# JuliaLinearAlgebra/IterativeSolvers.jl

Measured on AMD Instinct MI355X. Metric: cg_iters_per_sec, higher is better.
Workload: dtype f64; 1 GPU; cg! on 256^3 3D 7-point Laplacian (test/laplace_matrix.jl), fp64, hashed rhs, x0 = 0 (BASELINE.json configs[1]); n=16777216, nnz=117047296

## Files before the change

include/mik_dev.h:

```cpp
#include "mik.h"
#ifndef MIK_DEV_H
#define MIK_DEV_H
#ifdef __cplusplus
extern "C" {
#endif
enum {
    MIK_KNOB_LAYOUTS = 0,
    MIK_KNOB_CSR_KERNEL = 1,
    MIK_KNOB_SDIA_KERNEL = 2,
    MIK_KNOB_LONG_SEGMENT = 3,
    MIK_KNOB_UPLOAD = 4,
    MIK_KNOB_GS = 5,
    MIK_KNOB_TRANSPORT = 6,
    MIK_KNOB_NO_LOOKAHEAD = 7,
    MIK_KNOB_SOLVER_FORM = 8,
    MIK_KNOB_GS_TIMEOUT = 9,
    MIK_KNOB_CG_STEP = 10,
    MIK_KNOB_HOST_WAIT = 11,
    MIK_KNOB_MACHINE = 12,
    MIK_KNOB_COUNT = 13
};
int mik_set_tuning(int key, int value);
int mik_ctx_set_tuning(mik_ctx *ctx, int key, int value);
int mik_dev_gmres_form(const mik_gmres *it, int *single_launch, int *segments_per_workgroup, int *xcd_local_last, int *timeouts);
int mik_dev_dense_plan(const mik_dense *D, int adjoint, const void *x, const void *y, int *vec, int *streamed, int64_t *grid_x, int64_t *grid_y,
                       int64_t *chunks_or_batches, int64_t *segments);
int mik_dev_dense_block_plan(const mik_dense *D, int b, const void *X, int64_t ldx, const void *Y, int64_t ldy, int *vec, int *streamed,
                             int64_t *grid_x, int64_t *grid_y, int64_t *chunks, int *groups, int *last_width, int *vector_cols, int64_t *workspace_bytes);
int mik_dev_dense_block_min_width(mik_dense *D, int width);
int mik_dev_mgs_resident_shape(int *threads, int *register_rounds, int *lds_rounds);
int mik_dev_spmv_plan(const mik_csr *A, const void *x, int fuse_dot, int rb_begin, int rb_count, int skip_begin, int skip_end, char *kernel_name, int len,
                      int64_t *grid, int *launches, int *pre_longrows, int *post_rowdot);
int mik_dev_xwin_plan(int64_t n_blocks, const int *first_col, const int *last_col, const int *entries, int elem_size, int64_t n_cols,
                      int64_t total_entries, int *win_lo, int *span);
#ifdef __cplusplus
}
#endif
#endif
```

iterativesolvers.jl_amd/_lib.py:

```python
from __future__ import annotations

import ctypes as C
import os

import numpy as np

_HERE = os.path.dirname(os.path.abspath(__file__))
LIB_PATH = os.path.join(_HERE, "libmik.so")

MIK_OK = 0
MIK_F64, MIK_F32 = 0, 1
MIK_C64, MIK_C32 = 2, 3
MIK_SCALAR_REAL = 0x100
MIK_MGS, MIK_CGS, MIK_DGKS = 0, 1, 2
STATUS = {1: "invalid argument", 2: "HIP runtime error", 3: "dimension/dtype mismatch",
          4: "out of memory", 5: "not implemented", 6: "callback failed", 7: "norm outside the safely representable range",
          8: "singular"}


class MikError(RuntimeError):
    def __init__(self, code: int, where: str, detail: str = ""):
        self.code = code
        super().__init__(f"{where}: status {code} ({STATUS.get(code, '?')}) {detail}".rstrip())


_vp = C.c_void_p
_i64 = C.c_int64
_i64p = C.POINTER(C.c_int64)
_f64p = C.POINTER(C.c_double)
_ip = C.POINTER(C.c_int)

HALO_FN = C.CFUNCTYPE(C.c_int, C.c_void_p)
REDUCE_FN = C.CFUNCTYPE(C.c_int, C.c_void_p, C.c_int, C.c_int, C.c_void_p)


MUL_FN = C.CFUNCTYPE(C.c_int, C.c_void_p, C.c_void_p, C.c_void_p)
LDIV_FN = C.CFUNCTYPE(C.c_int, C.c_void_p, C.c_void_p, C.c_void_p)


class MikOperator(C.Structure):
    _fields_ = [("dtype", C.c_int), ("n", C.c_int64), ("csr", C.c_void_p), ("mul", MUL_FN), ("user", C.c_void_p)]


class MikPrecond(C.Structure):
    _fields_ = [("diag", C.c_void_p), ("ldiv", LDIV_FN), ("user", C.c_void_p)]


class MikDeviceInfo(C.Structure):
    _fields_ = [("device", C.c_int), ("compute_units", C.c_int), ("xcds", C.c_int), ("wavefront_size", C.c_int),
                ("lds_bytes_per_cu", C.c_int64), ("l2_bytes", C.c_int64), ("hbm_bytes", C.c_int64), ("arch", C.c_char * 64),
                ("planned_compute_units", C.c_int), ("planned_xcds", C.c_int), ("xcd_maps", C.c_int), ("resident_workgroup_cap", C.c_int),
                ("gs_single_launch_max_segments", C.c_int), ("gs_xcd_local_max_workgroups", C.c_int), ("sweep_grid_cap", C.c_int),
                ("mgs_resident_max_segments", C.c_int), ("reserved", C.c_int * 7)]


class MikPartition(C.Structure):
    _fields_ = [("rank", C.c_int), ("nranks", C.c_int), ("n_ext", C.c_int64), ("x_ext", C.c_void_p),
                ("send_idx", C.c_void_p), ("n_send", C.c_int64), ("send_buf", C.c_void_p),
                ("halo", HALO_FN), ("reduce", REDUCE_FN), ("user", C.c_void_p), ("link", C.c_void_p)]


class MikDensePlan(C.Structure):
    _fields_ = [("form", C.c_int), ("spin_limit", C.c_int)]


MIK_DENSE_AUTO, MIK_DENSE_PANEL, MIK_DENSE_CHAINED = 0, 1, 2


SIGNATURES = {
    "mik_abi_version": (C.c_int, []),
    "mik_device_count": (C.c_int, [_ip]),
    "mik_ctx_create": (C.c_int, [C.c_int, C.POINTER(_vp)]),
    "mik_ctx_destroy": (C.c_int, [_vp]),
    "mik_ctx_info": (C.c_int, [_vp, C.POINTER(MikDeviceInfo)]),
    "mik_dev_gmres_form": (C.c_int, [_vp, _ip, _ip, _ip, _ip]),
    "mik_dev_dense_plan": (C.c_int, [_vp, C.c_int, _vp, _vp, _ip, _ip, _i64p, _i64p, _i64p, _i64p]),
    "mik_dev_dense_block_plan": (C.c_int, [_vp, C.c_int, _vp, _i64, _vp, _i64, _ip, _ip, _i64p, _i64p, _i64p, _ip, _ip, _ip, _i64p]),
    "mik_dev_dense_block_min_width": (C.c_int, [_vp, C.c_int]),
    "mik_dev_mgs_resident_shape": (C.c_int, [_ip, _ip, _ip]),
    "mik_dev_spmv_plan": (C.c_int, [_vp, _vp, C.c_int, C.c_int, C.c_int, C.c_int, C.c_int, C.c_char_p, C.c_int, _i64p, _ip, _ip, _ip]),
    "mik_ctx_set_stream": (C.c_int, [_vp, _vp]),
    "mik_ctx_synchronize": (C.c_int, [_vp]),
    "mik_last_error": (C.c_char_p, [_vp]),
    "mik_reduce_shape": (C.c_int, [C.c_int, _ip, _ip]),
    "mik_spmv_dot_shape": (C.c_int, [_ip, _ip]),
    "mik_set_tuning": (C.c_int, [C.c_int, C.c_int]),
    "mik_ctx_set_tuning": (C.c_int, [_vp, C.c_int, C.c_int]),
    "mik_dev_xwin_plan": (C.c_int, [_i64, _ip, _ip, _ip, C.c_int, _i64, _i64, _ip, _ip]),
    "mik_spmv_long_row": (C.c_int, [_ip]),
    "mik_spmv_long_segment": (C.c_int, [_ip]),
    "mik_spmv_long_group": (C.c_int, [_ip]),
    "mik_malloc": (C.c_int, [_vp, C.c_size_t, C.POINTER(_vp)]),
    "mik_free": (C.c_int, [_vp, _vp]),
    "mik_memcpy_h2d": (C.c_int, [_vp, _vp, _vp, C.c_size_t]),
    "mik_memcpy_d2h": (C.c_int, [_vp, _vp, _vp, C.c_size_t]),
    "mik_copy": (C.c_int, [_vp, C.c_int, _i64, _vp, _vp]),
    "mik_fill": (C.c_int, [_vp, C.c_int, _i64, _vp, _vp]),
    "mik_csr_create": (C.c_int, [_vp, C.c_int, _i64, _i64, _i64, _i64p, _i64p, _vp, C.c_int, C.c_int,
                                 C.POINTER(_vp)]),
    "mik_csr_create_i32": (C.c_int, [_vp, C.c_int, _i64, _i64, _i64, C.POINTER(C.c_int32), C.POINTER(C.c_int32), _vp, C.c_int, C.c_int,
                                     C.POINTER(_vp)]),
    "mik_csr_destroy": (C.c_int, [_vp]),
    "mik_csr_layout": (C.c_int, [_vp, _ip]),
    "mik_csr_set_layout": (C.c_int, [_vp, C.c_int]),
    "mik_csr_stored_bytes": (C.c_int, [_vp, _i64p]),
    "mik_csr_compact": (C.c_int, [_vp]),
    "mik_spmv_kernel": (C.c_int, [_vp, C.c_char_p, C.c_int]),
    "mik_csr_info": (C.c_int, [_vp, _i64p, _i64p, _i64p, _ip]),
    "mik_spmv": (C.c_int, [_vp, _vp, _vp, _vp]),
    "mik_dot": (C.c_int, [_vp, C.c_int, _i64, _vp, _vp, _vp]),
    "mik_nrm2": (C.c_int, [_vp, C.c_int, _i64, _vp, _vp]),
    "mik_axpy": (C.c_int, [_vp, C.c_int, _i64, _vp, _vp, _vp]),
    "mik_xpby": (C.c_int, [_vp, C.c_int, _i64, _vp, _vp, _vp]),
    "mik_sub": (C.c_int, [_vp, C.c_int, _i64, _vp, _vp]),
    "mik_scal": (C.c_int, [_vp, C.c_int, _i64, _vp, _vp]),
    "mik_divide": (C.c_int, [_vp, C.c_int, _i64, _vp, _vp, _vp]),
    "mik_orthogonalize": (C.c_int, [_vp, C.c_int, _i64, C.c_int, _vp, _i64, _vp, _vp, _vp, C.c_int]),
    "mik_orthogonalize_vectors": (C.c_int, [_vp, C.c_int, _i64, C.c_int, C.POINTER(_vp), _vp, _vp, _vp]),
    "mik_gemv_n": (C.c_int, [_vp, C.c_int, _i64, C.c_int, _vp, _i64, _vp, _vp, _vp]),
    "mik_gemv_t": (C.c_int, [_vp, C.c_int, _i64, C.c_int, _vp, _i64, _vp, _vp]),
    "mik_lu_solve": (C.c_int, [C.c_int, _vp, _i64, C.c_int, _vp]),
    "mik_cg_create": (C.c_int, [_vp, _vp, _vp, _vp, _vp, _vp, _vp, _vp, C.c_double, C.c_double, _i64,
                                C.c_int, C.POINTER(_vp)]),
    "mik_cg_create_op": (C.c_int, [_vp, C.POINTER(MikOperator), C.POINTER(MikPrecond), _vp, _vp, _vp, _vp, _vp, C.c_double, C.c_double, _i64,
                                   C.c_int, C.POINTER(_vp)]),
    "mik_gmres_create_op": (C.c_int, [_vp, C.POINTER(MikOperator), C.POINTER(MikPrecond), C.POINTER(MikPrecond), _vp, _vp, C.c_double, C.c_double,
                                      C.c_int, _i64, C.c_int, C.c_int, C.POINTER(_vp)]),
    "mik_cg_destroy": (C.c_int, [_vp]),
    "mik_cg_fused_x": (C.c_int, [_vp, C.POINTER(C.c_int)]),
    "mik_cg_iterate": (C.c_int, [_vp, _i64, _f64p, _ip]),
    "mik_cg_iterate_many": (C.c_int, [_vp, _i64, _i64, _f64p, _i64p]),
    "mik_cg_state": (C.c_int, [_vp, _f64p, _f64p, _f64p, _i64p, _i64p, _ip]),
    "mik_gmres_create": (C.c_int, [_vp, _vp, _vp, _vp, _vp, _vp, C.c_double, C.c_double, C.c_int, _i64, C.c_int,
                                   C.c_int, C.POINTER(_vp)]),
    "mik_gmres_create_partitioned": (C.c_int, [_vp, _vp, _vp, _vp, _vp, _vp, C.c_double, C.c_double, C.c_int, _i64, C.c_int,
                                               C.c_int, C.POINTER(MikPartition), C.POINTER(_vp)]),
    "mik_gmres_destroy": (C.c_int, [_vp]),
    "mik_gmres_iterate": (C.c_int, [_vp, _i64, _f64p, _ip]),
    "mik_gmres_iterate_many": (C.c_int, [_vp, _i64, _i64, _f64p, _i64p]),
    "mik_gmres_state": (C.c_int, [_vp, _f64p, _f64p, _f64p, _ip, _i64p, _ip]),
    "mik_axpy_dot": (C.c_int, [_vp, C.c_int, _i64, _vp, _vp, _vp, _vp, _vp, C.c_int]),
    "mik_axpy2_nrm2": (C.c_int, [_vp, C.c_int, _i64, _vp, _vp, _vp, _vp, _vp, _vp, C.c_int]),
    "mik_cheb_direction": (C.c_int, [_vp, C.c_int, _i64, _vp, _vp, _vp, C.c_int, _vp]),
    "mik_minres_update": (C.c_int, [_vp, C.c_int, _i64, _vp, _vp, _vp, _vp, _vp, _vp, _vp, _vp, _vp, _vp, _vp, C.c_int]),
    "mik_gram": (C.c_int, [_vp, C.c_int, _i64, C.c_int, _vp, _i64, _vp]),
    "mik_bicgstab_mr_update": (C.c_int, [_vp, C.c_int, _i64, C.c_int, _vp, _i64, _vp, _i64, _vp, _vp, _vp]),
    "mik_bicgstab_create": (C.c_int, [_vp, _vp, C.c_int, _vp, _vp, _i64, _vp, _i64, _vp, _vp, C.POINTER(_vp)]),
    "mik_bicgstab_step": (C.c_int, [_vp, _vp]),
    "mik_bicgstab_destroy": (C.c_int, [_vp]),
    "mik_minres_create": (C.c_int, [_vp, _vp, _vp, _vp, _vp, _vp, _vp, _vp, _vp, C.c_double, C.c_int, C.POINTER(_vp)]),
    "mik_minres_step": (C.c_int, [_vp, _i64, _vp]),
    "mik_minres_proj_shape": (C.c_int, [_vp, _ip, _ip]),
    "mik_bicgstab_dot_shape": (C.c_int, [_vp, _ip, _ip]),
    "mik_minres_destroy": (C.c_int, [_vp]),
    "mik_xpby_nrm2": (C.c_int, [_vp, C.c_int, _i64, _vp, _vp, _vp, _vp]),
    "mik_lsqr_update": (C.c_int, [_vp, C.c_int, _i64, _vp, _vp, _vp, _vp, _vp, _vp, _vp]),
    "mik_lsmr_update": (C.c_int, [_vp, C.c_int, _i64, _vp, _vp, _vp, _vp, _vp, _vp, _vp, _vp]),
    "mik_axpy2_dot": (C.c_int, [_vp, C.c_int, _i64, _vp, _vp, _vp, _vp, _vp, _vp, _vp]),
    "mik_scal2": (C.c_int, [_vp, C.c_int, _i64, _vp, _vp, _vp, _vp]),
    "mik_qmr_update": (C.c_int, [_vp, C.c_int, _i64, _vp, _vp, _vp, _vp, _vp, _vp, _vp, _vp, _vp]),
    "mik_idrs_create": (C.c_int, [_vp, _vp, C.c_int, _vp, _vp, _vp, _i64, _vp, _i64, _vp, _i64, _vp, _vp, _vp, C.c_double, C.POINTER(_vp)]),
    "mik_idrs_step": (C.c_int, [_vp, C.c_int, _vp]),
    "mik_idrs_state": (C.c_int, [_vp, _vp, _vp, _vp]),
    "mik_idrs_destroy": (C.c_int, [_vp]),
    "mik_gather": (C.c_int, [_vp, C.c_int, _i64, _vp, _vp, _vp]),
    "mik_cgd_create": (C.c_int, [_vp, _vp, _vp, _vp, _vp, _vp, _vp, _vp, _i64, _vp, _vp, _vp, C.c_int, C.c_int,
                                 C.c_double, C.c_double, _i64, C.c_int, C.POINTER(_vp)]),
    "mik_cgd_destroy": (C.c_int, [_vp]),
    "mik_cgd_phase": (C.c_int, [_vp, C.c_int, _i64]),
    "mik_cgd_set_interior": (C.c_int, [_vp, _i64, _i64]),
    "mik_cgd_wait": (C.c_int, [_vp, _f64p, _f64p, _ip, _f64p, _i64, _i64p]),
    "mik_cgd_set_halo_plan": (C.c_int, [_vp, C.c_int, _ip, _i64p, _i64p, C.c_int, _ip, _i64p, _i64p]),
    "mik_cgd_halo_early": (C.c_int, [_vp, _ip, _i64p, _ip]),
    "mik_comm_unique_id": (C.c_int, [_vp]),
    "mik_comm_create": (C.c_int, [_vp, _vp, C.c_int, C.c_int, C.POINTER(_vp)]),
    "mik_comm_destroy": (C.c_int, [_vp]),
    "mik_comm_info": (C.c_int, [_vp, _ip, _ip, _ip]),
    "mik_comm_allgather_sum": (C.c_int, [_vp, C.c_int, C.c_int, _vp]),
    "mik_comm_halo": (C.c_int, [_vp, C.c_int, _vp, _vp, C.c_int, _ip, _i64p, _i64p, C.c_int, _ip, _i64p, _i64p]),
    "mik_cgd_set_comm": (C.c_int, [_vp, _vp]),
    "mik_comm_mailbox_export": (C.c_int, [_vp, _vp]),
    "mik_comm_mailbox_connect": (C.c_int, [_vp, _vp]),
    "mik_comm_mailbox_info": (C.c_int, [_vp, _ip, _ip]),
    "mik_cgd_ghost_export": (C.c_int, [_vp, _vp]),
    "mik_cgd_connect_ghosts": (C.c_int, [_vp, _vp, _i64p, _i64p]),
    "mik_plink_create": (C.c_int, [_vp, C.c_int, _i64, C.c_int, _ip, _i64p, _i64p, C.c_int, _ip, _i64p, _i64p, C.POINTER(_vp)]),
    "mik_plink_export": (C.c_int, [_vp, _vp]),
    "mik_plink_connect": (C.c_int, [_vp, _vp, _i64p, _i64p]),
    "mik_plink_info": (C.c_int, [_vp, _ip, _ip, _i64p]),
    "mik_plink_exchange": (C.c_int, [_vp, _vp, _vp]),
    "mik_plink_destroy": (C.c_int, [_vp]),
    "mik_cgd_init": (C.c_int, [_vp, _f64p, _f64p]),
    "mik_cgd_iterate_many": (C.c_int, [_vp, _i64, _i64, _f64p, _i64p]),
    "mik_cgd_group_init": (C.c_int, [C.POINTER(_vp), C.c_int, _f64p, _f64p]),
    "mik_cgd_group_iterate_many": (C.c_int, [C.POINTER(_vp), C.c_int, _i64, _i64, _f64p, _i64p]),
    "mik_cgd_group_release": (C.c_int, [C.POINTER(_vp), C.c_int]),
    "mik_hessenberg_ldiv": (C.c_int, [C.c_int, _vp, _i64, C.c_int, _vp]),
    "mik_givens": (C.c_int, [C.c_int, _vp, _vp, _vp]),
    "mik_time_spmv": (C.c_int, [_vp, _vp, _vp, _vp, C.c_int, C.c_int, _f64p]),
    "mik_cg_profile": (C.c_int, [_vp, C.c_int, _f64p, _i64p]),
    "mik_cgd_profile": (C.c_int, [_vp, C.c_int, _f64p, _i64p]),
    "mik_cg_profile_kernels": (C.c_int, [_vp, _f64p, _i64p]),
    "mik_stationary_create": (C.c_int, [_vp, _vp, _i64p, C.POINTER(_vp)]),
    "mik_stationary_destroy": (C.c_int, [_vp]),
    "mik_stationary_info": (C.c_int, [_vp, _i64p, _i64p, _i64p, _f64p]),
    "mik_diag_ldiv": (C.c_int, [_vp, _vp, _vp]),
    "mik_offdiag_mul": (C.c_int, [_vp, _vp, _vp, _vp, _vp]),
    "mik_gs_multiply": (C.c_int, [_vp, C.c_int, _vp, _vp, _vp, _vp, _vp]),
    "mik_forward_sub": (C.c_int, [_vp, _vp, _vp, _vp, _vp, C.c_int]),
    "mik_backward_sub": (C.c_int, [_vp, _vp, _vp, _vp, _vp, C.c_int]),
    "mik_dense_stationary_create": (C.c_int, [_vp, _vp, _i64, _i64, C.c_int, C.POINTER(MikDensePlan), _i64p, C.POINTER(_vp)]),
    "mik_dense_stationary_destroy": (C.c_int, [_vp]),
    "mik_dense_stationary_info": (C.c_int, [_vp, _i64p, _i64p, _i64p, _ip, _ip, _i64p]),
    "mik_dense_jacobi_step": (C.c_int, [_vp, _vp, _vp, _vp]),
    "mik_dense_gs_step": (C.c_int, [_vp, _vp, _vp]),
    "mik_dense_sor_step": (C.c_int, [_vp, _vp, _vp, _vp, _vp, C.c_int]),
    "mik_dense_ssor_step": (C.c_int, [_vp, _vp, _vp, _vp, _vp, C.c_int]),
    "mik_dense_mul_shape": (C.c_int, [_ip, _ip]),
    "mik_dense_mul_shape_for": (C.c_int, [C.c_int, _ip, _ip]),
    "mik_dense_create": (C.c_int, [_vp, C.c_int, _i64, _i64, _vp, _i64, C.POINTER(_vp)]),
    "mik_dense_destroy": (C.c_int, [_vp]),
    "mik_dense_mul": (C.c_int, [_vp, C.c_int, _vp, _vp]),
    "mik_dense_mm": (C.c_int, [_vp, C.c_int, _vp, _i64, _vp, _i64]),
    "mik_dense_block_reserve": (C.c_int, [_vp]),
    "mik_dense_block_shape": (C.c_int, [_ip]),
    "mik_dense_mul_fn": (C.c_int, [_vp, _vp, _vp]),
    "mik_dense_mul_adj_fn": (C.c_int, [_vp, _vp, _vp]),
    "mik_basis_rotate": (C.c_int, [_vp, C.c_int, _i64, C.c_int, C.c_int, _vp, _i64, _vp, _i64, _vp, _i64]),
    "mik_svdl_reorth": (C.c_int, [_vp, C.c_int, _i64, C.c_int, _vp, _i64, _vp, _vp, _vp, C.POINTER(C.c_int)]),
    "mik_spmm": (C.c_int, [_vp, _vp, C.c_int, _vp, _i64, _vp, _i64]),
    "mik_block_gram": (C.c_int, [_vp, C.c_int, _i64, C.c_int, C.c_int, _vp, _i64, _vp, _i64, _vp, _i64]),
    "mik_block_rdiv": (C.c_int, [_vp, C.c_int, _i64, C.c_int, _vp, _i64, _vp, _i64]),
    "mik_block_update": (C.c_int, [_vp, C.c_int, _i64, C.c_int, C.c_int, C.c_int, _vp, _i64, _vp, _i64, _vp, _i64, _vp, _i64, _vp, _i64, _vp, _i64]),
# ... 65 lines not shown
```

iterativesolvers.jl_amd/csrc/mik_core.hip:

```cpp
#include <algorithm>
#include <cmath>
#include <cstdarg>
#include <limits>
#include <new>

#include "mik_kernels.h"
#include "mik_spmv.h"
#include "mik_complex.h"
#include <algorithm>
#include <mutex>

#include "mik_sell.h"
#include "mik_jds.h"
#include <map>
#include <string>
#include <unordered_map>

thread_local std::string g_mik_create_error;
int g_mik_tuning[MIK_KNOB_COUNT] = {0};
static std::vector<mik_ctx *> g_mik_contexts;
static std::mutex g_mik_contexts_mu;

int mik_fail(mik_ctx *ctx, int code, const char *fmt, ...)
{
// ... 1474 lines not shown
    return lt;
}

template <typename T> static void spmv_go_sdiab(const SpmvPlan &p, const SpmvIO<T> &io)
{
    const mik_csr *A = io.A;
    with_consts([&](auto fd, auto cls) {
        constexpr int C = decltype(cls)::value;
        hipLaunchKernelGGL((k_spmv_sdiab<T, decltype(fd)::value, true, MIK_SDIAC_G, mik_sdiab_cls_ns(C), mik_sdiab_cls_cq(C)>), dim3(p.grid), dim3(MIK_BLOCK), 0,
                           io.ctx->stream, (int)A->n_rows, (int)A->n_cols, A->sdia_koff, p.rb0, p.nb, p.nfull, p.sshift, p.skip_at, p.skip_len,
                           (const SdiaSliceRec *)A->sdia_recs, (const SdiaPattern<T> *)A->sdia_pats, A->sdia_mask, io.x, io.y, io.seg_out, io.done);
    }, p.fd, SdiaCls{p.cls});
}

template <typename T> static void spmv_go_sdiab2(const SpmvPlan &p, const SpmvIO<T> &io)
{
    const mik_csr *A = io.A;
    with_consts([&](auto fd, auto cls) {
        constexpr int C = decltype(cls)::value;
        if constexpr (C >= 1)
            hipLaunchKernelGGL((k_spmv_sdiab2<T, decltype(fd)::value, true, mik_sdiab_cls_ns(C), mik_sdiab_cls_cq(C)>), dim3(p.grid), dim3(MIK_BLOCK), 0,
                               io.ctx->stream, (int)A->n_rows, (int)A->n_cols, A->sdia_koff, p.pb0, p.np, p.pfull, p.ps, p.nb_all,
                               (const SdiaSliceRec *)A->sdia_recs, (const SdiaPattern<T> *)A->sdia_pats, A->sdia_mask, io.x, io.y, io.seg_out, io.done,
                               io.ep_w(), io.ep_c(), io.ep_z());
    }, p.fd, SdiaCls{p.cls});
}

template <typename T> static void spmv_go_sdiac(const SpmvPlan &p, const SpmvIO<T> &io)
{
    const mik_csr *A = io.A;
    with_consts([&](auto fd) {
        hipLaunchKernelGGL((k_spmv_sdiac<T, decltype(fd)::value, true, MIK_SDIAC_G>), dim3(p.grid), dim3(MIK_BLOCK), 0, io.ctx->stream, (int)A->n_rows,
                           (int)A->n_cols, p.rb0, p.nb, p.map_mode, A->sdia_pat_id, (const SdiaPattern<T> *)A->sdia_pats, A->sdia_mask, io.x, io.y,
                           io.seg_out, io.done);
    }, p.fd);
}

template <typename T> static void spmv_go_sdiaw(const SpmvPlan &p, const SpmvIO<T> &io)
{
    const mik_csr *A = io.A;
    with_consts([&](auto fd) {
        if (p.kernel == SPMV_SDIAW2)
            hipLaunchKernelGGL((k_spmv_sdiaw2<T, decltype(fd)::value, true>), dim3(p.grid), dim3(MIK_BLOCK), 0, io.ctx->stream, (int)A->n_rows, (int)A->n_cols,
                               A->sdiaw_koff, p.pb0, p.np, p.pmode, p.nb_all, A->sdiaw_pat_id, (const SdiawPattern<T> *)A->sdiaw_pats, A->sdiaw_mask,
                               (const uint4 *)A->sdiaw_uz, io.x, io.y, io.seg_out, io.done);
        else
            hipLaunchKernelGGL((k_spmv_sdiaw<T, decltype(fd)::value, true>), dim3(p.grid), dim3(MIK_BLOCK), 0, io.ctx->stream, (int)A->n_rows, A->sdiaw_koff,
                               p.rb0, p.nb, p.map_mode, A->sdiaw_pat_id, (const SdiawPattern<T> *)A->sdiaw_pats, A->sdiaw_mask, io.x, io.y, io.seg_out,
                               io.done);
    }, p.fd);
}

template <typename T> static void spmv_go_sdia(const SpmvPlan &p, const SpmvIO<T> &io)
{
    const mik_csr *A = io.A;
    with_consts([&](auto fd) {
        hipLaunchKernelGGL((k_spmv_sdia<T, decltype(fd)::value, true>), dim3(p.grid), dim3(MIK_BLOCK), 0, io.ctx->stream, (int)A->n_rows, (int)A->n_cols, p.rb0,
                           p.nb, p.map_mode, A->sdia_ptr, A->sdia_off, A->sdia_tri, A->sdia_mask, (const T *)A->sdia_val, io.x, io.y, io.seg_out, io.done);
    }, p.fd);
}

template <typename T> static void spmv_go_jds(const SpmvPlan &p, const SpmvIO<T> &io)
{
    const mik_csr *A = io.A;
    using IV = typename WideVec<T>::idx;
    using VV = typename WideVec<T>::val;
    with_consts([&](auto fd, auto mg) {
        if constexpr (!(decltype(fd)::value && decltype(mg)::value))
            hipLaunchKernelGGL((k_spmv_jds<T, decltype(fd)::value, true, decltype(mg)::value>), dim3(p.grid), dim3(MIK_BLOCK), 0, io.ctx->stream, (int)A->n_rows,
                               p.rb0, A->jds_ptr, A->jds_len, (const IV *)A->jds_col, (const VV *)A->jds_val, io.x, io.y, io.seg_out, io.done, p.nlb,
                               spmv_long_tab(A), A->col, (const T *)A->val, io.ep_w(), io.ep_c(), io.ep_z());
    }, p.fd, p.merge);
}

template <typename T> static void spmv_go_rowgather(const SpmvPlan &p, const SpmvIO<T> &io)
{
    const mik_csr *A = io.A;
    with_consts([&](auto fd) {
        hipLaunchKernelGGL((k_spmv_rowgather<T, decltype(fd)::value, true>), dim3(p.grid), dim3(MIK_BLOCK), 0, io.ctx->stream, (int)A->n_rows, p.rb0, p.nb,
                           p.map_mode, A->rowptr, A->col, (const T *)A->val, io.x, io.y, io.seg_out, io.done, A->is_long, io.ep_w(), io.ep_c(), io.ep_z());
    }, p.fd);
}

template <typename T> static void spmv_go_rowblock(const SpmvPlan &p, const SpmvIO<T> &io)
{
    const mik_csr *A = io.A;
    with_consts([&](auto fd, auto mg, auto nt, auto xw, auto rp) {
        if constexpr (!(decltype(fd)::value && decltype(mg)::value))
            hipLaunchKernelGGL((k_spmv_rowblock<T, decltype(fd)::value, decltype(nt)::value, true, decltype(mg)::value, decltype(xw)::value, decltype(rp)::value>),
                               dim3(p.grid), dim3(MIK_BLOCK), p.lds, io.ctx->stream, (int)A->n_rows, p.nb, p.map_mode, A->rowptr, A->col, (const T *)A->val,
                               io.x, io.y, io.seg_out, io.done, A->is_long, p.nlb, spmv_long_tab(A), (const int *)A->xwin_lo, A->xwin_span,
                               (const unsigned char *)A->rperm, (p.merge && p.long_win) ? (const int *)A->long_win : (const int *)nullptr, p.lw_launch,
                               io.ep_w(), io.ep_c(), io.ep_z());
    }, p.fd, p.merge, p.nt_rb, p.xwin, p.rp);
}

template <typename T> static int spmv_run(const SpmvPlan &p, const SpmvIO<T> &io)
{
    mik_ctx *ctx = io.ctx;
    const mik_csr *A = io.A;
    if (p.rc != MIK_OK) return mik_fail(ctx, p.rc, "%s", p.refusal);
    if (p.empty) return MIK_OK;
    if (p.pre_longrows) {
        hipLaunchKernelGGL((k_spmv_longrows<T>), dim3(p.nlb), dim3(MIK_BLOCK), p.pre_lds, ctx->stream, spmv_long_tab(A), A->col, (const T *)A->val, io.x, io.y,
                           io.done, p.long_win ? (const int *)A->long_win : (const int *)nullptr, A->long_lw);
        MIK_LAUNCH_CHECK(ctx);
    }
    switch (p.kernel) {
    case SPMV_ROWGATHER: spmv_go_rowgather<T>(p, io); break;
    case SPMV_ROWBLOCK: spmv_go_rowblock<T>(p, io); break;
    case SPMV_JDS: spmv_go_jds<T>(p, io); break;
    case SPMV_SDIA: spmv_go_sdia<T>(p, io); break;
    case SPMV_SDIAC: spmv_go_sdiac<T>(p, io); break;
    case SPMV_SDIAB: spmv_go_sdiab<T>(p, io); break;
    case SPMV_SDIAB2: spmv_go_sdiab2<T>(p, io); break;
    case SPMV_SDIAW: case SPMV_SDIAW2: spmv_go_sdiaw<T>(p, io); break;
    }
    MIK_LAUNCH_CHECK(ctx);
    if (p.post_rowdot) {
        hipLaunchKernelGGL((k_rowdot<T>), dim3(p.nb_all), dim3(MIK_BLOCK), 0, ctx->stream, (int)A->n_rows, io.x, (const T *)io.y, io.seg_out, io.done);
        MIK_LAUNCH_CHECK(ctx);
    }
    return MIK_OK;
}

template <typename T>
int mik_spmv_launch_range(mik_ctx *ctx, const mik_csr *A, const T *x, T *y, bool fuse_dot, T *seg_out, const int *done, int rb_begin,
                          int rb_count)
{
    return spmv_run<T>(spmv_plan(A, sizeof(T), mik_aligned16(x), fuse_dot, rb_begin, rb_count, SPMV_NO_SKIP, 0, spmv_ep_armed(ctx)), {ctx, A, x, y, seg_out, done});
}

template <typename T>
int mik_spmv_launch(mik_ctx *ctx, const mik_csr *A, const T *x, T *y, bool fuse_dot, T *seg_out, const int *done)
{
    return mik_spmv_launch_range<T>(ctx, A, x, y, fuse_dot, seg_out, done, 0, -1);
}

template <typename T>
int mik_spmv_launch_outside(mik_ctx *ctx, const mik_csr *A, const T *x, T *y, bool fuse_dot, T *seg_out, const int *done, int skip_begin, int skip_end)
{
    SpmvPlan p[2];
    const int np = spmv_plan_outside(A, sizeof(T), mik_aligned16(x), fuse_dot, skip_begin, skip_end, spmv_ep_armed(ctx), p);
    for (int i = 0; i < np; ++i) MIK_TRY(spmv_run<T>(p[i], {ctx, A, x, y, seg_out, done}));
    return MIK_OK;
}
template int mik_spmv_launch_outside<double>(mik_ctx *, const mik_csr *, const double *, double *, bool, double *, const int *, int, int);
template int mik_spmv_launch_outside<float>(mik_ctx *, const mik_csr *, const float *, float *, bool, float *, const int *, int, int);
template int mik_spmv_launch<double>(mik_ctx *, const mik_csr *, const double *, double *, bool, double *, const int *);
template int mik_spmv_launch<float>(mik_ctx *, const mik_csr *, const float *, float *, bool, float *, const int *);
template int mik_spmv_launch_range<double>(mik_ctx *, const mik_csr *, const double *, double *, bool, double *, const int *, int, int);
template int mik_spmv_launch_range<float>(mik_ctx *, const mik_csr *, const float *, float *, bool, float *, const int *, int, int);

extern "C" int mik_spmv(mik_ctx *ctx, const mik_csr *A, const void *x, void *y)
{
    if (!ctx || !A || !x || !y) return MIK_ERR_INVALID;
    if (x == y) return mik_fail(ctx, MIK_ERR_INVALID, "mik_spmv: x and y must not alias");
    if (mik_is_complex(A->dtype)) return mik_c_spmv(ctx, A, x, y);
    return A->dtype == MIK_F64 ? mik_spmv_launch<double>(ctx, A, (const double *)x, (double *)y, false, nullptr, nullptr)
                               : mik_spmv_launch<float>(ctx, A, (const float *)x, (float *)y, false, nullptr, nullptr);
}

template <typename T>
static int time_spmv_impl(mik_ctx *ctx, const mik_csr *A, const void *x, void *y, int fused, int reps, double *avg_ms)
{
    int rc = mik_ensure_partials(ctx, sizeof(T) * (size_t)std::max<int64_t>((A->n_rows + MIK_BLOCK - 1) / MIK_BLOCK, 1));
    if (rc) return rc;
    hipEvent_t e0, e1;
    MIK_HIP(ctx, hipEventCreate(&e0));
    MIK_HIP(ctx, hipEventCreate(&e1));
    MIK_HIP(ctx, hipEventRecord(e0, ctx->stream));
    for (int i = 0; i < reps; ++i) {
        rc = mik_spmv_launch<T>(ctx, A, (const T *)x, (T *)y, fused != 0, (T *)ctx->partials, nullptr);
        if (rc) return rc;
    }
    MIK_HIP(ctx, hipEventRecord(e1, ctx->stream));
    MIK_HIP(ctx, hipEventSynchronize(e1));
    float ms = 0.f;
    MIK_HIP(ctx, hipEventElapsedTime(&ms, e0, e1));
    (void)hipEventDestroy(e0);
    (void)hipEventDestroy(e1);
    *avg_ms = (double)ms / reps;
    return MIK_OK;
}

extern "C" int mik_time_spmv(mik_ctx *ctx, const mik_csr *A, const void *x, void *y, int fused_dot, int reps, double *avg_ms)
{
    if (!ctx || !A || !x || !y || reps <= 0 || !avg_ms) return MIK_ERR_INVALID;
    if (mik_is_complex(A->dtype)) return mik_c_time_spmv(ctx, A, x, y, reps, avg_ms);
    return A->dtype == MIK_F64 ? time_spmv_impl<double>(ctx, A, x, y, fused_dot, reps, avg_ms)
                               : time_spmv_impl<float>(ctx, A, x, y, fused_dot, reps, avg_ms);
}

template <typename T> static int reduce_to_host(mik_ctx *ctx, int64_t n, T *out)
{
    const int64_t nseg = mik_nseg<T>(n);
    hipLaunchKernelGGL((k_finalize_store<T>), dim3(1), dim3(MIK_FIN_THREADS), 0, ctx->stream, (const T *)ctx->partials, nseg,
                       (int64_t)0, (T *)ctx->coef, (const int *)nullptr);
    MIK_LAUNCH_CHECK(ctx);
    return mik_read_scalars<T>(ctx, (const T *)ctx->coef, 1, out);
}

template <typename T> static int norm_from_sumsq(mik_ctx *ctx, int64_t n, const T *x, T t, T *out)
{
    if (mik_nrm_in_range(t)) { *out = (T)std::sqrt(t); return MIK_OK; }
    return mik_safe_norm_slow<T>(ctx, n, x, out);
}

template <typename T> int mik_safe_norm_slow(mik_ctx *ctx, int64_t n, const T *x, T *out)
{
    if (n <= 0) { *out = T(0); return MIK_OK; }
    T *scr = (T *)((unsigned char *)ctx->coef + mik_ctx::COEF_SAFE_SLOT);
    const int grid = (int)std::min<int64_t>((n + MIK_BLOCK - 1) / MIK_BLOCK, 1024);
    MIK_TRY(mik_ensure_partials(ctx, sizeof(T) * (size_t)std::max<int64_t>(std::max<int64_t>(mik_nseg<T>(n), grid), 1)));
    hipLaunchKernelGGL((k_amax<T>), dim3(grid), dim3(MIK_BLOCK), 0, ctx->stream, n, x, (T *)ctx->partials);
    MIK_LAUNCH_CHECK(ctx);
    hipLaunchKernelGGL((k_amax<T>), dim3(1), dim3(MIK_BLOCK), 0, ctx->stream, (int64_t)grid, (const T *)ctx->partials, scr);
    MIK_LAUNCH_CHECK(ctx);
    T amax;
    MIK_TRY(mik_read_scalars<T>(ctx, scr, 1, &amax));
    T sc, sinv;
    if (!mik_nrm_scale(amax, sc, sinv)) { *out = amax; return MIK_OK; }
    OpScaledSq<T> op{x, sc};
    MIK_TRY((launch_map<T>(ctx, n, op, mik_aligned16(x), (T *)ctx->partials, nullptr)));
    hipLaunchKernelGGL((k_finalize_store<T>), dim3(1), dim3(MIK_FIN_THREADS), 0, ctx->stream, (const T *)ctx->partials, mik_nseg<T>(n),
                       (int64_t)0, scr, (const int *)nullptr);
    MIK_LAUNCH_CHECK(ctx);
    T t2;
    MIK_TRY(mik_read_scalars<T>(ctx, scr, 1, &t2));
    *out = (T)std::sqrt(t2) * sinv;
    return MIK_OK;
}
template int mik_safe_norm_slow<double>(mik_ctx *, int64_t, const double *, double *);
template int mik_safe_norm_slow<float>(mik_ctx *, int64_t, const float *, float *);

template <typename T> static int dot_impl(mik_ctx *ctx, int64_t n, const void *x, const void *y, void *out, bool nrm)
{
    int rc = mik_ensure_partials(ctx, sizeof(T) * (size_t)std::max<int64_t>(mik_nseg<T>(n), 1));
    if (rc) return rc;
    OpDot<T> op{(const T *)x, (const T *)y};
    rc = launch_map<T>(ctx, n, op, mik_aligned16(x) && mik_aligned16(y), (T *)ctx->partials, nullptr);
    if (rc) return rc;
    T v;
    MIK_TRY(reduce_to_host<T>(ctx, n, &v));
    if (!nrm) { *(T *)out = v; return MIK_OK; }
    return norm_from_sumsq<T>(ctx, n, (const T *)x, v, (T *)out);
}

extern "C" int mik_dot(mik_ctx *ctx, int dtype, int64_t n, const void *x, const void *y, void *out)
{
    if (!ctx || n < 0 || !out || (n && (!x || !y))) return MIK_ERR_INVALID;
    if (mik_is_complex(dtype)) return mik_c_dot(ctx, dtype, n, x, y, out);
    return dtype == MIK_F64 ? dot_impl<double>(ctx, n, x, y, out, false) : dot_impl<float>(ctx, n, x, y, out, false);
}

extern "C" int mik_nrm2(mik_ctx *ctx, int dtype, int64_t n, const void *x, void *out)
{
    if (!ctx || n < 0 || !out || (n && !x)) return MIK_ERR_INVALID;
    if (mik_is_complex(dtype)) return mik_nrm2(ctx, mik_real_dtype(dtype), 2 * n, x, out);
    return dtype == MIK_F64 ? dot_impl<double>(ctx, n, x, x, out, true) : dot_impl<float>(ctx, n, x, x, out, true);
}

extern "C" int mik_axpy(mik_ctx *ctx, int dtype, int64_t n, const void *alpha, const void *x, void *y)
{
    if (!ctx || n < 0 || !alpha || (n && (!x || !y))) return MIK_ERR_INVALID;
    if (mik_is_complex(dtype & ~MIK_SCALAR_REAL))
        return (dtype & MIK_SCALAR_REAL) ? mik_axpy(ctx, mik_real_dtype(dtype & ~MIK_SCALAR_REAL), 2 * n, alpha, x, y) : mik_c_axpy(ctx, dtype, n, alpha, x, y);
    const bool vec = mik_aligned16(x) && mik_aligned16(y);
    if (dtype == MIK_F64) { OpAxpy<double> op{(const double *)x, (double *)y, coef_val(*(const double *)alpha)}; return launch_map<double>(ctx, n, op, vec, (double *)nullptr, nullptr); }
    if (dtype == MIK_F32) { OpAxpy<float> op{(const float *)x, (float *)y, coef_val(*(const float *)alpha)}; return launch_map<float>(ctx, n, op, vec, (float *)nullptr, nullptr); }
    return MIK_ERR_INVALID;
}

extern "C" int mik_xpby(mik_ctx *ctx, int dtype, int64_t n, const void *x, const void *beta, void *y)
{
    if (!ctx || n < 0 || !beta || (n && (!x || !y))) return MIK_ERR_INVALID;
    if (mik_is_complex(dtype & ~MIK_SCALAR_REAL))
        return (dtype & MIK_SCALAR_REAL) ? mik_xpby(ctx, mik_real_dtype(dtype & ~MIK_SCALAR_REAL), 2 * n, x, beta, y) : mik_c_xpby(ctx, dtype, n, x, beta, y);
    const bool vec = mik_aligned16(x) && mik_aligned16(y);
    if (dtype == MIK_F64) { OpXpby<double> op{(const double *)x, (double *)y, coef_val(*(const double *)beta)}; return launch_map<double>(ctx, n, op, vec, (double *)nullptr, nullptr); }
    if (dtype == MIK_F32) { OpXpby<float> op{(const float *)x, (float *)y, coef_val(*(const float *)beta)}; return launch_map<float>(ctx, n, op, vec, (float *)nullptr, nullptr); }
    return MIK_ERR_INVALID;
}

extern "C" int mik_sub(mik_ctx *ctx, int dtype, int64_t n, const void *x, void *y)
{
    if (!ctx || n < 0 || (n && (!x || !y))) return MIK_ERR_INVALID;
    if (mik_is_complex(dtype)) return mik_sub(ctx, mik_real_dtype(dtype), 2 * n, x, y);
    const bool vec = mik_aligned16(x) && mik_aligned16(y);
    if (dtype == MIK_F64) { OpSub<double> op{(const double *)x, (double *)y}; return launch_map<double>(ctx, n, op, vec, (double *)nullptr, nullptr); }
    if (dtype == MIK_F32) { OpSub<float> op{(const float *)x, (float *)y}; return launch_map<float>(ctx, n, op, vec, (float *)nullptr, nullptr); }
    return MIK_ERR_INVALID;
}

extern "C" int mik_scal(mik_ctx *ctx, int dtype, int64_t n, const void *alpha, void *x)
{
    if (!ctx || n < 0 || !alpha || (n && !x)) return MIK_ERR_INVALID;
    if (mik_is_complex(dtype & ~MIK_SCALAR_REAL))
        return (dtype & MIK_SCALAR_REAL) ? mik_scal(ctx, mik_real_dtype(dtype & ~MIK_SCALAR_REAL), 2 * n, alpha, x) : mik_c_scal(ctx, dtype, n, alpha, x);
    const bool vec = mik_aligned16(x);
    if (dtype == MIK_F64) { OpScal<double> op{(double *)x, coef_val(*(const double *)alpha)}; return launch_map<double>(ctx, n, op, vec, (double *)nullptr, nullptr); }
    if (dtype == MIK_F32) { OpScal<float> op{(float *)x, coef_val(*(const float *)alpha)}; return launch_map<float>(ctx, n, op, vec, (float *)nullptr, nullptr); }
    return MIK_ERR_INVALID;
}

template <typename T>
// ... 221 lines not shown
```

iterativesolvers.jl_amd/csrc/mik_spmv.h:

```cpp
#pragma once
#include "mik_internal.h"

#ifdef __HIPCC__

template <bool NT, typename U> __device__ __forceinline__ U ld_stream(const U *p)
{
    return NT ? __builtin_nontemporal_load(p) : *p;
}
template <bool NT, typename U> __device__ __forceinline__ void st_stream(U *p, U v)
{
    if (NT) __builtin_nontemporal_store(v, p); else *p = v;
}

typedef double mik_f64x2 __attribute__((ext_vector_type(2)));
typedef float mik_f32x4 __attribute__((ext_vector_type(4)));
typedef int mik_i32x2 __attribute__((ext_vector_type(2)));
typedef int mik_i32x4 __attribute__((ext_vector_type(4)));
template <typename T> struct WideVec;
template <> struct WideVec<double> { using val = mik_f64x2; using idx = mik_i32x2; };
template <> struct WideVec<float>  { using val = mik_f32x4; using idx = mik_i32x4; };

__device__ __forceinline__ int spmv_block_map(int b, int nb, int mode)
{
    if (mode == 1) return xcd_remap(b, nb);
// ... 152 lines not shown
    constexpr int TILE = MIK_SPMV_TILE * (int)(8 / sizeof(T));
    constexpr int VW = WIDE ? VT<T>::W : 1;
    constexpr int PER = TILE / (MIK_BLOCK * VW);
    extern __shared__ __attribute__((aligned(16))) unsigned char mik_dyn_lds[];
    T *prod = reinterpret_cast<T *>(mik_dyn_lds);
    T *lds4 = prod + TILE + 8;

    const int t = threadIdx.x;
    int bid = blockIdx.x;
    if (MERGE_LONG) {
        const bool spread = lw < 0;
        if (spread) lw = -lw;
        unsigned which = (unsigned)bid;
        bool is_long = bid < nlb;
        if (spread) {
            const unsigned total = gridDim.x;
            const unsigned before = (unsigned)(((unsigned long long)bid * (unsigned)nlb + total - 1) / total);
            const unsigned upto = (unsigned)(((unsigned long long)(bid + 1) * (unsigned)nlb + total - 1) / total);
            is_long = upto > before;
            which = is_long ? before : (unsigned)bid - before;
        } else if (!is_long) which = (unsigned)(bid - nlb);
        if (is_long) {
            const int lwlo = long_win ? long_win[which] : -1;
            if (lwlo >= 0) spmv_long_window<T>(x, prod, lwlo, lw);
            spmv_longrow_wave<T>((int)which * (MIK_BLOCK / 64) + (t >> 6), lt, col, val, x, y, prod, lwlo >= 0 ? lwlo : 0, lwlo >= 0 ? lw : 0);
            return;
        }
        bid = (int)which;
    }
    const int rb = spmv_block_map(bid, nb, map_mode);
    const int r0 = rb * MIK_BLOCK;
    const int tr = RPERM ? (int)rperm[r0 + t] : t;
    const int r = r0 + tr;
    int ks = 0, ke = 0;
    if (r < n) { ks = rowptr[r]; ke = rowptr[r + 1]; }
    const int kb = rowptr[r0] & ~(VW - 1);
    const int kend = rowptr[min(r0 + MIK_BLOCK, n)];
    T *xw = lds4 + 16 / (int)sizeof(T) * ((4 * (int)sizeof(T) + 15) / 16);
    int wlo = 0;
    if (XWIN) {
        constexpr int XP = 1024 / (int)sizeof(T);
        wlo = win_lo[rb];
        if (kb < kend && wlo >= 0)
            for (int piece = t >> 6; piece * XP < win_span; piece += MIK_BLOCK / 64)
                __builtin_amdgcn_global_load_lds((const __attribute__((address_space(1))) void *)(x + wlo + piece * XP + (t & 63) * (16 / (int)sizeof(T))),
                                                 (__attribute__((address_space(3))) void *)(xw + piece * XP), 16, 0, 0);
    }

    T acc = T(0);
    for (int kc = kb; kc < kend; kc += TILE) {
        const int cnt = min(TILE, kend - kc);
        if (WIDE) {
            using VV = typename WideVec<T>::val;
            using IV = typename WideVec<T>::idx;
            VV v[PER];
            IV c[PER];
#pragma unroll
            for (int i = 0; i < PER; ++i) {
                const int j = VW * (t + MIK_BLOCK * i);
                if (j < cnt) {
                    v[i] = ld_stream<NT>(reinterpret_cast<const VV *>(val + kc + j));
                    c[i] = ld_stream<NT>(reinterpret_cast<const IV *>(col + kc + j));
                }
            }
            if (XWIN && wlo >= 0) {
                if (kc == kb) {
                    asm volatile("s_waitcnt vmcnt(0)" ::: "memory");
                    __syncthreads();
                }
#pragma unroll
                for (int i = 0; i < PER; ++i) {
                    const int j = VW * (t + MIK_BLOCK * i);
                    if (j < cnt) {
#pragma unroll
                        for (int e = 0; e < VW; ++e) {
                            const unsigned o = min((unsigned)(c[i][e] - wlo), (unsigned)(win_span - 1));
                            prod[j + e] = v[i][e] * xw[o];
                        }
                    }
                }
            } else {
#pragma unroll
                for (int i = 0; i < PER; ++i) {
                    const int j = VW * (t + MIK_BLOCK * i);
                    if (j < cnt) {
                        T xv[VW];
#pragma unroll
                        for (int e = 0; e < VW; ++e) xv[e] = x[c[i][e]];
#pragma unroll
                        for (int e = 0; e < VW; ++e) prod[j + e] = v[i][e] * xv[e];
                    }
                }
            }
        } else {
            T v[PER];
            int c[PER];
#pragma unroll
            for (int i = 0; i < PER; ++i) {
                const int j = t + MIK_BLOCK * i;
                if (j < cnt) { v[i] = ld_stream<NT>(val + kc + j); c[i] = ld_stream<NT>(col + kc + j); }
            }
#pragma unroll
            for (int i = 0; i < PER; ++i) {
                const int j = t + MIK_BLOCK * i;
                if (j < cnt) prod[j] = v[i] * x[c[i]];
            }
        }
        __syncthreads();
        int a = max(ks, kc) - kc;
        int len = min(ke, kc + cnt) - kc - a;
        for (; len >= 8; len -= 8, a += 8) {
            T q[8];
#pragma unroll
            for (int i = 0; i < 8; ++i) q[i] = prod[a + i];
#pragma unroll
            for (int i = 0; i < 8; ++i) acc = acc + q[i];
        }
        if (len > 0) {
            T q[8];
#pragma unroll
            for (int i = 0; i < 8; ++i) q[i] = prod[a + i];
#pragma unroll
            for (int i = 0; i < 8; ++i) {
                const T s2 = acc + q[i];
                acc = i < len ? s2 : acc;
            }
        }
        __syncthreads();
    }
    if (FUSE_DOT && ep_w && r < n) { const T te = *ep_c * ep_w[r]; acc = acc + te; }
    if (is_long && r < n && is_long[r]) acc = y[r];
    else if (r < n) st_stream<NT>(y + r, acc);
    if (FUSE_DOT) {
        T p = T(0);
        if (r < n) p = (ep_z ? ep_z[r] : x[r]) * acc;
        if (RPERM) {
            prod[tr] = p;
            __syncthreads();
            p = prod[t];
        }
        T tot = block_tree_256(p, lds4);
        if (t == 0) seg_out[rb] = tot;
    }
}

template <typename T, bool FUSE_DOT, bool NT>
__global__ __launch_bounds__(MIK_BLOCK, 6) void k_spmv_rowgather(int n, int rb0, int nb, int map_mode, const int *__restrict__ rowptr,
                                                              const int *__restrict__ col, const T *__restrict__ val,
                                                              const T *__restrict__ x, T *__restrict__ y, T *__restrict__ seg_out,
                                                              const int *__restrict__ done, const unsigned char *__restrict__ is_long,
                                                              const T *__restrict__ ep_w = nullptr, const T *__restrict__ ep_c = nullptr,
                                                             const T *__restrict__ ep_z = nullptr)
{
    if (done && *done) return;
    constexpr int TILE = MIK_SPMV_TILE;
    constexpr int VW = VT<T>::W;
    constexpr int VP = 1024 / (int)sizeof(T);
    constexpr int CP = 256;
    __shared__ __attribute__((aligned(16))) T sval[TILE];
    __shared__ __attribute__((aligned(16))) int scol[TILE];
    __shared__ T lds4[4];

    const int t = threadIdx.x, lane = t & 63, wv = t >> 6;
    const int rb = rb0 + spmv_block_map((int)blockIdx.x, nb, map_mode);
    const int r0 = rb * MIK_BLOCK;
    const int r = r0 + t;
    int ks = 0, ke = 0;
    if (r < n) { ks = rowptr[r]; ke = rowptr[r + 1]; }
    const int kb = rowptr[r0] & ~3;
    const int kend = rowptr[min(r0 + MIK_BLOCK, n)];

    T acc = T(0);
    for (int kc = kb; kc < kend; kc += TILE) {
        const int cnt = min(TILE, kend - kc);
#pragma unroll
        for (int p = 0; p < TILE / VP / 4; ++p) {
            const int piece = wv + 4 * p;
            if (piece * VP < cnt)
                __builtin_amdgcn_global_load_lds((const __attribute__((address_space(1))) void *)(val + kc + piece * VP + lane * VW),
                                                 (__attribute__((address_space(3))) void *)(sval + piece * VP), 16, 0, NT ? 2 : 0);
        }
#pragma unroll
        for (int p = 0; p < TILE / CP / 4; ++p) {
            const int piece = wv + 4 * p;
            if (piece * CP < cnt)
                __builtin_amdgcn_global_load_lds((const __attribute__((address_space(1))) void *)(col + kc + piece * CP + lane * 4),
                                                 (__attribute__((address_space(3))) void *)(scol + piece * CP), 16, 0, NT ? 2 : 0);
        }
        asm volatile("s_waitcnt vmcnt(0)" ::: "memory");
        __syncthreads();
        int a = max(ks, kc) - kc;
        int len = min(ke, kc + cnt) - kc - a;
        while (len > 0) {
            T q[8];
            int cc[8];
#pragma unroll
            for (int i = 0; i < 8; ++i) {
                const int s = min(a + i, TILE - 1);
                cc[i] = scol[s];
                q[i] = sval[s];
            }
#pragma unroll
            for (int i = 0; i < 8; ++i) {
                const T xv = x[i < len ? cc[i] : 0];
                q[i] = q[i] * xv;
            }
#pragma unroll
            for (int i = 0; i < 8; ++i)
                if (i < len) acc = acc + q[i];
            a += 8;
            len -= 8;
        }
        if (kc + TILE < kend) __syncthreads();
    }
    if (FUSE_DOT && ep_w && r < n) { const T te = *ep_c * ep_w[r]; acc = acc + te; }
    if (is_long && r < n && is_long[r]) acc = y[r];
    else if (r < n) st_stream<NT>(y + r, acc);
    if (FUSE_DOT) {
        T p = T(0);
        if (r < n) p = (ep_z ? ep_z[r] : x[r]) * acc;
        T tot = block_tree_256(p, lds4);
        if (t == 0) seg_out[rb] = tot;
    }
}

#endif
```

Baseline: 2166 iters/s.

## Pipeline rowgather SpMV tile loads: issue col before val, overlap x gather

The row-gather SpMV kernel now issues the column-index LDS loads before the value loads and waits only for the column loads. It then starts the first batch of x gathers before waiting for the value tile, so value loading overlaps with the dependent x reads. Row pointers, the done flag and the fused-dot operand are loaded up front, pinned in registers, and the dot reuses the prefetched x value. The change also adds a C/Python entry point, mik_dev_spmv_run, for launching SpMV ranges directly. In exchange it relies on hand-managed vmcnt/barrier sequencing and adds an extra barrier per tile, which raises the risk of correctness bugs.

```diff
diff --git a/include/mik_dev.h b/include/mik_dev.h
--- a/include/mik_dev.h
+++ b/include/mik_dev.h
@@ -31,6 +31,8 @@
 int mik_dev_mgs_resident_shape(int *threads, int *register_rounds, int *lds_rounds);
 int mik_dev_spmv_plan(const mik_csr *A, const void *x, int fuse_dot, int rb_begin, int rb_count, int skip_begin, int skip_end, char *kernel_name, int len,
                       int64_t *grid, int *launches, int *pre_longrows, int *post_rowdot);
+int mik_dev_spmv_run(mik_ctx *ctx, const mik_csr *A, const void *x, void *y, int fuse_dot, void *seg_out, int rb_begin, int rb_count, int skip_begin,
+                     int skip_end);
 int mik_dev_xwin_plan(int64_t n_blocks, const int *first_col, const int *last_col, const int *entries, int elem_size, int64_t n_cols,
                       int64_t total_entries, int *win_lo, int *span);
 #ifdef __cplusplus
diff --git a/iterativesolvers.jl_amd/_lib.py b/iterativesolvers.jl_amd/_lib.py
--- a/iterativesolvers.jl_amd/_lib.py
+++ b/iterativesolvers.jl_amd/_lib.py
@@ -79,6 +79,7 @@
     "mik_dev_dense_block_min_width": (C.c_int, [_vp, C.c_int]),
     "mik_dev_mgs_resident_shape": (C.c_int, [_ip, _ip, _ip]),
     "mik_dev_spmv_plan": (C.c_int, [_vp, _vp, C.c_int, C.c_int, C.c_int, C.c_int, C.c_int, C.c_char_p, C.c_int, _i64p, _ip, _ip, _ip]),
+    "mik_dev_spmv_run": (C.c_int, [_vp, _vp, _vp, _vp, C.c_int, _vp, C.c_int, C.c_int, C.c_int, C.c_int]),
     "mik_ctx_set_stream": (C.c_int, [_vp, _vp]),
     "mik_ctx_synchronize": (C.c_int, [_vp]),
     "mik_last_error": (C.c_char_p, [_vp]),
diff --git a/iterativesolvers.jl_amd/csrc/mik_core.hip b/iterativesolvers.jl_amd/csrc/mik_core.hip
--- a/iterativesolvers.jl_amd/csrc/mik_core.hip
+++ b/iterativesolvers.jl_amd/csrc/mik_core.hip
@@ -1650,6 +1650,24 @@
 template int mik_spmv_launch_range<double>(mik_ctx *, const mik_csr *, const double *, double *, bool, double *, const int *, int, int);
 template int mik_spmv_launch_range<float>(mik_ctx *, const mik_csr *, const float *, float *, bool, float *, const int *, int, int);
 
+template <typename T>
+static int dev_spmv_run(mik_ctx *ctx, const mik_csr *A, const void *x, void *y, bool fuse_dot, void *seg_out, int rb_begin, int rb_count, int skip_begin,
+                        int skip_end)
+{
+    if (skip_begin < 0) return mik_spmv_launch_range<T>(ctx, A, (const T *)x, (T *)y, fuse_dot, (T *)seg_out, nullptr, rb_begin, rb_count);
+    return mik_spmv_launch_outside<T>(ctx, A, (const T *)x, (T *)y, fuse_dot, (T *)seg_out, nullptr, skip_begin, skip_end);
+}
+
+extern "C" int mik_dev_spmv_run(mik_ctx *ctx, const mik_csr *A, const void *x, void *y, int fuse_dot, void *seg_out, int rb_begin, int rb_count,
+                                int skip_begin, int skip_end)
+{
+    if (!ctx || !A || !x || !y || (fuse_dot && !seg_out)) return MIK_ERR_INVALID;
+    if (x == y) return mik_fail(ctx, MIK_ERR_INVALID, "mik_dev_spmv_run: x and y must not alias");
+    MIK_REFUSE_COMPLEX(ctx, A, "mik_dev_spmv_run");
+    return A->dtype == MIK_F64 ? dev_spmv_run<double>(ctx, A, x, y, fuse_dot != 0, seg_out, rb_begin, rb_count, skip_begin, skip_end)
+                               : dev_spmv_run<float>(ctx, A, x, y, fuse_dot != 0, seg_out, rb_begin, rb_count, skip_begin, skip_end);
+}
+
 extern "C" int mik_spmv(mik_ctx *ctx, const mik_csr *A, const void *x, void *y)
 {
     if (!ctx || !A || !x || !y) return MIK_ERR_INVALID;
diff --git a/iterativesolvers.jl_amd/csrc/mik_spmv.h b/iterativesolvers.jl_amd/csrc/mik_spmv.h
--- a/iterativesolvers.jl_amd/csrc/mik_spmv.h
+++ b/iterativesolvers.jl_amd/csrc/mik_spmv.h
@@ -328,7 +328,6 @@
                                                               const T *__restrict__ ep_w = nullptr, const T *__restrict__ ep_c = nullptr,
                                                              const T *__restrict__ ep_z = nullptr)
 {
-    if (done && *done) return;
     constexpr int TILE = MIK_SPMV_TILE;
     constexpr int VW = VT<T>::W;
     constexpr int VP = 1024 / (int)sizeof(T);
@@ -337,25 +336,27 @@
     __shared__ __attribute__((aligned(16))) int scol[TILE];
     __shared__ T lds4[4];
 
-    const int t = threadIdx.x, lane = t & 63, wv = t >> 6;
+    const int t = threadIdx.x, lane = t & 63;
+    const int wv = __builtin_amdgcn_readfirstlane(t >> 6);
     const int rb = rb0 + spmv_block_map((int)blockIdx.x, nb, map_mode);
     const int r0 = rb * MIK_BLOCK;
     const int r = r0 + t;
-    int ks = 0, ke = 0;
-    if (r < n) { ks = rowptr[r]; ke = rowptr[r + 1]; }
-    const int kb = rowptr[r0] & ~3;
+    const int rl = min(r, n - 1);
+    int ks = rowptr[rl], ke = rowptr[rl + 1];
+    T xr = T(0);
+    if (FUSE_DOT) xr = (ep_z ? ep_z : x)[rl];
+    const int kfirst = rowptr[r0];
     const int kend = rowptr[min(r0 + MIK_BLOCK, n)];
+    const int stop = *(done ? done : rowptr);
+    if (FUSE_DOT) asm volatile("" :: "v"(ks), "v"(ke), "v"(xr), "s"(kfirst), "s"(kend), "s"(stop), "s"(col), "s"(val), "s"(x), "s"(y));
+    else asm volatile("" :: "v"(ks), "v"(ke), "s"(kfirst), "s"(kend), "s"(stop), "s"(col), "s"(val), "s"(x), "s"(y));
+    if (done && stop) return;
+    if (r >= n) ks = ke = 0;
+    const int kb = kfirst & ~3;
 
     T acc = T(0);
     for (int kc = kb; kc < kend; kc += TILE) {
         const int cnt = min(TILE, kend - kc);
-#pragma unroll
-        for (int p = 0; p < TILE / VP / 4; ++p) {
-            const int piece = wv + 4 * p;
-            if (piece * VP < cnt)
-                __builtin_amdgcn_global_load_lds((const __attribute__((address_space(1))) void *)(val + kc + piece * VP + lane * VW),
-                                                 (__attribute__((address_space(3))) void *)(sval + piece * VP), 16, 0, NT ? 2 : 0);
-        }
 #pragma unroll
         for (int p = 0; p < TILE / CP / 4; ++p) {
             const int piece = wv + 4 * p;
@@ -363,10 +364,50 @@
                 __builtin_amdgcn_global_load_lds((const __attribute__((address_space(1))) void *)(col + kc + piece * CP + lane * 4),
                                                  (__attribute__((address_space(3))) void *)(scol + piece * CP), 16, 0, NT ? 2 : 0);
         }
-        asm volatile("s_waitcnt vmcnt(0)" ::: "memory");
-        __syncthreads();
+        int nv = 0;
+#pragma unroll
+        for (int p = 0; p < TILE / VP / 4; ++p) {
+            const int piece = wv + 4 * p;
+            if (piece * VP < cnt) {
+                __builtin_amdgcn_global_load_lds((const __attribute__((address_space(1))) void *)(val + kc + piece * VP + lane * VW),
+                                                 (__attribute__((address_space(3))) void *)(sval + piece * VP), 16, 0, NT ? 2 : 0);
+                ++nv;
+            }
+        }
+        if (nv >= 4) asm volatile("s_waitcnt vmcnt(4)" ::: "memory");
+        else if (nv == 3) asm volatile("s_waitcnt vmcnt(3)" ::: "memory");
+        else if (nv == 2) asm volatile("s_waitcnt vmcnt(2)" ::: "memory");
+        else if (nv == 1) asm volatile("s_waitcnt vmcnt(1)" ::: "memory");
+        else asm volatile("s_waitcnt vmcnt(0)" ::: "memory");
+        asm volatile("s_waitcnt lgkmcnt(0)" ::: "memory");
+        __builtin_amdgcn_s_barrier();
+        asm volatile("" ::: "memory");
         int a = max(ks, kc) - kc;
         int len = min(ke, kc + cnt) - kc - a;
+        {
+            T q[8], xv[8];
+            int cc[8];
+#pragma unroll
+            for (int i = 0; i < 8; ++i) cc[i] = scol[min(a + i, TILE - 1)];
+#pragma unroll
+            for (int i = 0; i < 8; ++i) {
+                xv[i] = T(0);
+                if (__builtin_amdgcn_ballot_w64(i < len) != 0) xv[i] = x[i < len ? cc[i] : 0];
+            }
+            asm volatile("s_waitcnt vmcnt(0)"
+                         : "+v"(xv[0]), "+v"(xv[1]), "+v"(xv[2]), "+v"(xv[3]), "+v"(xv[4]), "+v"(xv[5]), "+v"(xv[6]), "+v"(xv[7])
+                         :: "memory");
+            asm volatile("s_waitcnt lgkmcnt(0)" ::: "memory");
+            __builtin_amdgcn_s_barrier();
+            asm volatile("" ::: "memory");
+#pragma unroll
+            for (int i = 0; i < 8; ++i) q[i] = sval[min(a + i, TILE - 1)] * xv[i];
+#pragma unroll
+            for (int i = 0; i < 8; ++i)
+                if (i < len) acc = acc + q[i];
+            a += 8;
+            len -= 8;
+        }
         while (len > 0) {
             T q[8];
             int cc[8];
@@ -394,7 +435,7 @@
     else if (r < n) st_stream<NT>(y + r, acc);
     if (FUSE_DOT) {
         T p = T(0);
-        if (r < n) p = (ep_z ? ep_z[r] : x[r]) * acc;
+        if (r < n) p = xr * acc;
         T tot = block_tree_256(p, lds4);
         if (t == 0) seg_out[rb] = tot;
     }
```

Result: faster. 2219 iters/s, median of 6 (+2.4%).
